# agent-charon/MinGraph-UNet

Hardware: AMD Instinct MI355X
Metric: segmented Mpix/sec, full MinGraph-UNet forward (U-Net + patch-graph GAT), 512x512 batch (higher is better)
Workload: dtype f32

## Files before the change

include/mgunet.h:

```cpp
#ifndef MGUNET_H
#define MGUNET_H

#include <stddef.h>
#include <stdint.h>

#ifdef __cplusplus
extern "C" {
#endif

#define MGU_OK 0
#define MGU_ERR_INVALID -1
#define MGU_ERR_HIP -2
#define MGU_ERR_STATE -3
#define MGU_ERR_NOMEM -4

#define MGU_DTYPE_F32 0
#define MGU_DTYPE_BF16 1

typedef struct mgu_ctx mgu_ctx;

typedef struct {
  const char* name;
  const void* ptr;
  int64_t numel;
// ... 318 lines not shown
int mgu_refine_probs(mgu_ctx* ctx, const float* src_dev, int is_prob, const uint8_t* guide_dev, int B, int H, int W, int C, int G, int radius,
                     const int32_t* space_lut, const int32_t* range_lut, int shift, int iterations, float* probs_dev, int64_t* labels_dev,
                     float* conf_dev, int64_t* changed_dev, void* hip_stream);
int mgu_slic_labels(mgu_ctx* ctx, const uint8_t* rgb_dev, int B, int H, int W, int step, int mq, int passes, const uint16_t* lin_host,
                    const int32_t* m_host, const uint16_t* f_host, int32_t* raw_labels_dev, int32_t* centres_dev, void* hip_stream);
int mgu_regions_connect(mgu_ctx* ctx, const int32_t* raw_labels_dev, int B, int H, int W, int min_area, int rounds, int32_t* labels_dev,
                        int64_t* counts_dev, int64_t* offsets_dev, void* hip_stream);
int mgu_regions_adjacency(mgu_ctx* ctx, const int32_t* labels_dev, const int64_t* offsets_dev, int B, int H, int W, int64_t node_capacity,
                          int64_t edge_capacity, int32_t* rowptr_dev, int32_t* col_dev, int32_t* border_dev, int32_t* status_dev,
                          void* hip_stream);
int mgu_regions_features_u8(mgu_ctx* ctx, const uint8_t* rgb_dev, const int32_t* labels_dev, const int64_t* offsets_dev, int B, int H, int W,
                            const uint16_t* lin_host, const int32_t* m_host, const uint16_t* f_host, int64_t node_capacity, float* feat_dev,
                            int64_t* stats_dev, void* hip_stream);
int mgu_regions_pool_nhwc(mgu_ctx* ctx, const float* feat_dev, int ld, int c_off, int D, const int32_t* labels_dev, const int64_t* offsets_dev,
                          int B, int H, int W, int64_t node_capacity, float* out_dev, void* hip_stream);
int mgu_patch_node_features_u8(mgu_ctx* ctx, const uint8_t* rgb_dev, int B, int H, int W, int patch, const float* img_dev, int64_t is_n,
                               int64_t is_c, int64_t is_h, int64_t is_w, int repeat, const float* unet_rows_dev, int unet_cols, int per_channel,
                               float* out_dev, int ld_out, void* hip_stream);
int mgu_patch_labels(mgu_ctx* ctx, const void* src_dev, int src_kind, int B, int H, int W, int C, int patch, int32_t* counts_dev,
                     int64_t* labels_dev, float* purity_dev, void* hip_stream);
int mgu_graphcut_rev_index(mgu_ctx* ctx, const int64_t* coo_dev, int64_t E, int num_nodes, const int32_t* rowptr_dev, const int32_t* col_dev,
                           int32_t* rev_dev, int32_t* perm_dev, int* status_dev, void* hip_stream);
int mgu_graphcut_capacities(mgu_ctx* ctx, int B, int N, const int64_t* coo_dev, int64_t E, const float* prior_dev, const int32_t* counts_dev,
                            int num_classes, int fg_class, const float* intensity_dev, const float* feat_dev, int D, float gamma,
                            float sigma_intensity, float sigma_features, float smoothness, float unit, int32_t* cap_source_dev,
                            int32_t* cap_sink_dev, int32_t* cap_edge_dev, void* hip_stream);
int mgu_graphcut_solve(mgu_ctx* ctx, int B, int N, int64_t E, const int32_t* rowptr_dev, const int32_t* col_dev, const int32_t* rev_dev,
                       const int32_t* perm_dev, const int32_t* cap_source_dev, const int32_t* cap_sink_dev, const int32_t* cap_edge_dev,
                       int max_rounds, int relabel_period, int threads, uint8_t* labels_dev, int64_t* flow_dev, int32_t* rounds_dev,
                       int32_t* converged_dev, void* hip_stream);
int mgu_graphcut_energy(mgu_ctx* ctx, int B, int N, const int64_t* coo_dev, int64_t E, const uint8_t* labels_dev, const int32_t* cap_source_dev,
                        const int32_t* cap_sink_dev, const int32_t* cap_edge_dev, int64_t* energy_dev, void* hip_stream);
int mgu_graphcut_label_costs(mgu_ctx* ctx, int64_t rows, int K, const float* prob_dev, const int32_t* counts_dev, float unit, int32_t* costs_dev,
                             void* hip_stream);
int mgu_graphcut_expand(mgu_ctx* ctx, int B, int N, int64_t E, int K, const int32_t* rowptr_dev, const int32_t* col_dev, const int32_t* rev_dev,
                        const int32_t* perm_dev, const int32_t* costs_dev, const int32_t* cap_edge_dev, const uint8_t* init_dev, int max_cycles,
                        int max_rounds, int relabel_period, int threads, uint8_t* labels_dev, int64_t* energy_dev, int32_t* moves_dev,
                        int32_t* accepted_dev, int32_t* rounds_dev, int32_t* converged_dev, void* hip_stream);
int mgu_graphcut_energy_multi(mgu_ctx* ctx, int B, int N, const int64_t* coo_dev, int64_t E, int K, const uint8_t* labels_dev, const int32_t* costs_dev,
                              const int32_t* cap_edge_dev, int64_t* energy_dev, void* hip_stream);
int mgu_colorize_labels(mgu_ctx* ctx, const int64_t* labels_dev, int64_t npix, const uint8_t* palette_dev, int num_classes, uint8_t* vis_dev,
                        uint8_t* labels_u8_dev, void* hip_stream);

int mgu_channel_affine_nhwc(mgu_ctx* ctx, const float* x_dev, int ldx, int64_t M, int C, const float* scale_dev,
                            const float* shift_dev, int act, float* y_dev, int ldy, void* hip_stream);
int mgu_channel_sum_nhwc(mgu_ctx* ctx, const float* x_dev, int ldx, int64_t M, int C, float* out_dev, void* hip_stream);

int mgu_channel_sum_images_nhwc(mgu_ctx* ctx, const float* x_dev, int ldx, int B, int64_t M, int C, float* out_dev, void* hip_stream);

int mgu_frame_sad_tile(void);
int mgu_frame_shifts(mgu_ctx* ctx, const uint8_t* frames_u8, int T, int H, int W, int channels, int bgr, int radius, int factor,
                     int32_t* shifts_dev, int64_t* cost_dev, int64_t* surface_dev, void* hip_stream);
int mgu_track_align(mgu_ctx* ctx, const int32_t* labels_dev, const int64_t* offsets_dev, int64_t capacity, const int32_t* shifts_dev, int T,
                    int H, int W, int32_t* prev_aligned_dev, int32_t* next_cropped_dev, int64_t* vis_prev_dev, int64_t* vis_next_dev,
                    void* hip_stream);
int mgu_track_ids(mgu_ctx* ctx, const int64_t* offsets_dev, int T, int64_t capacity, const int64_t* link_dev, const int64_t* class_dev,
                  const int64_t* first_ids_dev, int64_t* next_id_dev, int64_t* track_id_dev, int32_t* track_len_dev, int64_t* track_class_dev,
                  int64_t track_capacity, int32_t* status_dev, void* hip_stream);

int mgu_mask_runs(mgu_ctx* ctx, const int32_t* labels_dev, const int64_t* offsets_dev, int64_t capacity, int B, int H, int W,
                  int64_t run_capacity, int64_t* run_ptr_dev, int32_t* run_start_dev, int32_t* run_length_dev, int32_t* status_dev,
                  void* hip_stream);
int mgu_runs_to_labels(mgu_ctx* ctx, const int64_t* run_ptr_dev, const int32_t* run_start_dev, const int32_t* run_length_dev,
                       int64_t run_capacity, const int64_t* offsets_dev, int64_t capacity, int B, int H, int W, int32_t* labels_dev,
                       int32_t* status_dev, void* hip_stream);
int mgu_object_outlines(mgu_ctx* ctx, const int32_t* labels_dev, const int64_t* offsets_dev, int64_t capacity, int B, int H, int W,
                        int connectivity, int64_t loop_capacity, int64_t vertex_capacity, int64_t* loop_ptr_dev, int64_t* vertex_ptr_dev,
                        int32_t* vertices_dev, int64_t* loop_area2_dev, int32_t* status_dev, void* hip_stream);
int mgu_polygons_to_labels(mgu_ctx* ctx, const int64_t* loop_ptr_dev, const int64_t* vertex_ptr_dev, const int32_t* vertices_dev,
                           int64_t loop_capacity, int64_t vertex_capacity, const int64_t* offsets_dev, int64_t capacity, int B, int H, int W,
                           int frac_bits, int64_t crossing_capacity, int32_t* labels_dev, int32_t* status_dev, void* hip_stream);

double mgu_unet_flops(mgu_ctx* ctx, int B, int H, int W);
double mgu_unet_mfma_flops(mgu_ctx* ctx, int B, int H, int W);
int mgu_profile_enable(mgu_ctx* ctx, int on);
typedef struct {
  const char* name;
  double ms, flops_alg, flops_mfma;
  int launches, pipe;
} mgu_kernel_stat;
int mgu_profile_read_kernels(mgu_ctx* ctx, mgu_kernel_stat* out, int cap, int* n_out);
int mgu_profile_read(mgu_ctx* ctx, double* conv_ms, int* conv_launches, double* total_ms);
int64_t mgu_convt_asm_launches(mgu_ctx* ctx);

#ifdef __cplusplus
}
#endif
#endif
```

mingraph-unet_amd/csrc/common.h:

```cpp
#pragma once
#include <hip/hip_runtime.h>
#include <stdint.h>

#include "device.h"

namespace mgu {

inline int grid_for(int64_t work, int threads, int cap) {
  int64_t b = (work + threads - 1) / threads;
  if (b < 1) b = 1;
  if (b > cap) b = cap;
  return (int)b;
}
inline bool aligned16(const void* p) { return ((uintptr_t)p & 15) == 0; }

struct Tuning {
  bool first_mfma = true;
  bool use_wino = true;
  int wino_prec = 1;
  bool convt_frag = true;
  bool wino_cp = true;
  int wino_ppb_cap = 32;
  bool wgrad_halo = true;
  bool wino_wgrad = true;
  bool convt_dgrad_x3 = true;
  bool wgrad_x3 = true;
  bool wgrad_thin = true;
  bool wino_dgrad = true;
  bool gat_fused = true;
  bool head_fused = true;
  bool wino_asm = true;
  bool convt_asm = true;
  int fwd_groups = 2;
  int lovasz_passes = 4;
};
const Tuning& default_tuning();
hipError_t ensure_dyn_lds(const void* func, size_t bytes, bool (&done)[64]);

struct IgemmDesc {
  const Tuning* tn;
  const float* in;
  const float* w;
  const float* wu;
  const float* scale;
  const float* shift;
  float* out;
  int M;
  int H, W;
  int Cp;
  int ldin;
  int KS;
  int K;
  int Kp;
  int N;
  int ldout;
  int coff;
  int relu;
  int out_mode;
  int ct_cout;
  int Hout, Wout;
  float* pool;
  int ldpool;
  double* stat_slots;
  int split_n;
  float* out2;
  int ld2;
};

struct WinoHead {
  const float* w;
  const float* b;
  float* logits;
  float* psum;
  int ncls;
  int psum_bytes;
};
inline size_t wino_head_psum_bytes(int B, int H, int W) { return (size_t)B * (H / 16) * (W / 16) * 8 * 32 * sizeof(float); }

inline const Tuning& tun(const IgemmDesc& d) { return d.tn ? *d.tn : default_tuning(); }
enum class ConvKernel {
  None,
  WinoAsmWide, WinoAsmCp1r2, WinoAsmCp1r4,
  WinoAsmCp1r2Head,
  WinoCp2, WinoCp1, WinoCp2Stats, WinoCp1Stats,
  WinoCp1Head,
  WinoF32Wide, WinoF32Narrow,
  WinoX3Wide, WinoX3Narrow,
  HaloF32, HaloBf16Np8, HaloBf16Np4,
  TilesF32, TilesBf16,
  ConvtX3, ConvtBf16f, ConvtX3Dgrad,
  ConvtX3Asm,
};
ConvKernel pick_conv(const IgemmDesc& d, int dtype, const WinoHead* head = nullptr);
hipError_t launch_conv(const IgemmDesc& d, ConvKernel k, int dtype, hipStream_t s, const WinoHead* head = nullptr);
inline bool conv_fuses_head(ConvKernel k) { return k == ConvKernel::WinoAsmCp1r2Head || k == ConvKernel::WinoCp1Head; }
inline hipError_t launch_igemm_f32(const IgemmDesc& d, hipStream_t s) { return launch_conv(d, pick_conv(d, 0), 0, s); }
inline hipError_t launch_igemm_bf16(const IgemmDesc& d, hipStream_t s) { return launch_conv(d, pick_conv(d, 1), 1, s); }
const char* conv_kernel_name(ConvKernel k, const IgemmDesc& d);
const char* conv_dgrad_name(ConvKernel k, const IgemmDesc& d);
struct ConvCost {
  double mfma;
  int pipe;
};
ConvCost conv_cost(ConvKernel k, const IgemmDesc& d);
inline bool conv_is_wino(ConvKernel k) { return k >= ConvKernel::WinoAsmWide && k <= ConvKernel::WinoX3Narrow; }
inline bool conv_fuses_pool(ConvKernel k) {
  return conv_is_wino(k) || (k >= ConvKernel::HaloF32 && k <= ConvKernel::HaloBf16Np4);
}
inline bool conv_reads_panel(ConvKernel k) {
  return !conv_is_wino(k) && k != ConvKernel::ConvtX3 && k != ConvKernel::ConvtX3Asm && k != ConvKernel::ConvtBf16f &&
         k != ConvKernel::ConvtX3Dgrad;
}
inline bool conv_reads_convt_x3(ConvKernel k) {
  return k == ConvKernel::ConvtX3 || k == ConvKernel::ConvtX3Asm;
}
bool wino_layer(const Tuning& t, int KS, int Cp);
// ... 165 lines not shown
```

mingraph-unet_amd/csrc/ctx.h:

```cpp
#pragma once
#include <stdarg.h>
#include <stdio.h>
#include <stdlib.h>
#include <string.h>

#include <map>
#include <string>
#include <vector>

#include "../../include/mgunet.h"
#include "common.h"

struct Layer {
  std::string prefix;
  std::string conv;
  std::string bn;
  int Cin = 0, Cp = 0, Cout = 0, KS = 3;
  bool convt = false;
  int K = 0, Kp = 0, N = 0, Np = 0;
  float *wp = nullptr, *scale = nullptr, *shift = nullptr;
  bool first = false;
  bool ctb = false;
  bool ctx3 = false;
  bool wino = false;
// ... 17 lines not shown
  int ldin = 0;
  float* z = nullptr;
  float* y = nullptr;
  int ldy = 0;
  int B = 0, H = 0, W = 0;
};

struct Block {
  int up = -1;
  int conv1 = 0, conv2 = 0;
  int level = 0;
};

struct mgu_ctx {
  int device = 0;
  mgu::Tuning tn;
  std::string err;
  bool configured = false, loaded = false;
  std::vector<mgu::PackBatch> pack_host;
  mgu::PackBatch* pack_dev = nullptr;
  int pack_dev_cap = 0;
  bool want_train = false;
  bool fold_dirty = false;
  int* err_word = nullptr;
  void* redws = nullptr;
  size_t redws_bytes = 0;
  void* pm_out = nullptr;
  int pm_patch = 0;
  void* pmws = nullptr;
  size_t pmws_bytes = 0;
  void* wuws = nullptr;
  size_t wuws_bytes = 0;
  unsigned long long* gmaxbuf = nullptr;
  int gmax_cap = 0;
  unsigned gmax_gen = 0;
  struct mgu_gat_weights* gat_tmp = nullptr;
  void* lossws = nullptr;
  size_t lossws_bytes = 0;
  void* optws = nullptr;
  size_t optws_bytes = 0;
  void* imgws = nullptr;
  size_t imgws_bytes = 0;
  void* ncws = nullptr;
  size_t ncws_bytes = 0;
  void* objws = nullptr;
  size_t objws_bytes = 0;
  void* labtab = nullptr;
  std::vector<unsigned char> labtab_host;
  int in_ch = 0, ncls = 0, feat = 0, depth = 0, dtype = 0, Cp0 = 0;
  std::vector<Layer> layers;
  std::vector<Block> enc, dec;
  Block bott;
  int head = 0;
  int64_t nparams = 0;
  float* arena = nullptr;
  size_t arena_floats = 0;
  void* ws = nullptr;
  size_t ws_bytes = 0;
  void* gbws = nullptr;
  size_t gbws_bytes = 0;
  void* gws = nullptr;
  size_t gws_bytes = 0;
  void* tws = nullptr;
  size_t tws_bytes = 0;
  bool have_train_fwd = false;
  int tB = 0, tH = 0, tW = 0;
  std::vector<FwdRecord> fwd;
  void* comm = nullptr;
  int comm_world = 1, comm_rank = 0;
  hipStream_t comm_stream = nullptr;
  hipEvent_t comm_ev[16] = {};
  int comm_ev_next = 0;
  bool prof = false;
  std::vector<hipEvent_t> ev;
  struct ProfRec {
    const char* name;
    double alg, mfma;
    int pipe;
  };
  std::vector<ProfRec> prec;
  int ev_used = 0;
  hipEvent_t ev_total[2] = {nullptr, nullptr};
  hipStream_t fwd_stream = nullptr;
  hipEvent_t fwd_ev[2] = {nullptr, nullptr};
  int64_t convt_asm_launches = 0;
  int panel_packs = 0;
};

namespace mgud {

inline int rup(int v, int m) { return (v + m - 1) / m * m; }
extern std::string g_create_err;

inline Layer make_layer(int dtype, int Cin, int Cp, int Cout, int KS, bool convt) {
  Layer L;
  L.Cin = Cin, L.Cp = Cp, L.Cout = Cout, L.KS = KS, L.convt = convt;
  L.K = KS * KS * Cp, L.Kp = rup(L.K, dtype == MGU_DTYPE_BF16 ? 64 : 32);
  L.N = convt ? 4 * Cout : Cout, L.Np = rup(L.N, 128);
  return L;
}

inline int fail(mgu_ctx* c, int code, const char* fmt, ...) {
  char buf[512];
  va_list ap;
  va_start(ap, fmt);
  vsnprintf(buf, sizeof buf, fmt, ap);
  va_end(ap);
  if (c) c->err = buf; else g_create_err = buf;
  return code;
}

#define HIPCHK(c, call)                                                                                       \
  do {                                                                                                        \
    hipError_t e_ = (call);                                                                                   \
    if (e_ != hipSuccess) return mgud::fail(c, MGU_ERR_HIP, "%s failed: %s", #call, hipGetErrorString(e_));   \
  } while (0)

inline int ensure(mgu_ctx* c, void** p, size_t* have, size_t need) {
  if (*have >= need) return MGU_OK;
  if (*p) {
    HIPCHK(c, hipDeviceSynchronize());
    HIPCHK(c, hipFree(*p));
    *p = nullptr;
    *have = 0;
  }
  hipError_t e = hipMalloc(p, need);
  if (e != hipSuccess) return fail(c, MGU_ERR_NOMEM, "hipMalloc(%zu) failed: %s", need, hipGetErrorString(e));
  *have = need;
  return MGU_OK;
}

inline int err_word_dev(mgu_ctx* c, int** dev) {
  if (!c->err_word) {
    HIPCHK(c, hipHostMalloc((void**)&c->err_word, sizeof(int), hipHostMallocMapped));
    *c->err_word = 0;
  }
  HIPCHK(c, hipHostGetDevicePointer((void**)dev, c->err_word, 0));
  return MGU_OK;
}
inline const char* err_word_message(int w) {
  return (w & 2) ? "the GAT backward found no edge whose score equals the forward's graph-wide maximum (mgu_gat_layer_backward): its "
                   "max term was not applied"
                 : "a label outside [0, num_classes) (and != ignore_index -100) reached a loss kernel of this context (mgu_cross_entropy / "
                   "mgu_dice_loss; F.one_hot / CrossEntropyLoss raise on it)";
}

struct Carve {
  size_t off = 0;
  size_t take(size_t bytes) {
    const size_t o = off;
    off += (bytes + 255) / 256 * 256;
    return o;
  }
};

struct ProfScope {
  mgu_ctx* c;
  hipStream_t s;
  int idx = -1;
  ProfScope(mgu_ctx* c_, hipStream_t s_, const char* name = "conv/GEMM", double alg = 0, double mfma = 0, int pipe = -1) : c(c_), s(s_) {
    if (!c || !c->prof) return;
    if ((size_t)c->ev_used >= c->prec.size()) c->prec.resize(c->ev_used + 1);
    c->prec[c->ev_used] = {name, alg, mfma, pipe};
    if ((size_t)(2 * c->ev_used + 2) > c->ev.size()) {
      hipEvent_t a, b;
      if (hipEventCreate(&a) != hipSuccess || hipEventCreate(&b) != hipSuccess) return;
      c->ev.push_back(a);
// ... 141 lines not shown
```

mingraph-unet_amd/csrc/mgunet_api.hip:

```cpp
#include "ctx.h"

#include <algorithm>

using namespace mgu;
using namespace mgud;

namespace mgud {
std::string g_create_err;
}

namespace {

struct WsPlan {
  size_t xin, tmp, tmp_slice, bott, total;
  std::vector<size_t> pooled;
};

int fwd_groups(const mgu_ctx* c, int B) { return c->tn.fwd_groups >= 2 && B >= 2 ? 2 : 1; }
int group_images(const mgu_ctx* c, int B) { return (B + fwd_groups(c, B) - 1) / fwd_groups(c, B); }

WsPlan plan_ws(const mgu_ctx* c, int B, int H, int W) {
  std::vector<int> hs, wsz;
  level_dims(H, W, c->depth, hs, wsz);
  auto out = [&](const Block& b, int l) { return (size_t)B * hs[l] * wsz[l] * c->layers[b.conv2].Cout; };
  WsPlan p;
  Carve k;
  const size_t es = c->dtype == MGU_DTYPE_BF16 ? 2 : 4;
  p.xin = k.take((size_t)B * H * W * c->Cp0 * es);
  size_t tmax = out(c->bott, c->bott.level);
  for (const Block& b : c->enc) tmax = std::max(tmax, out(b, b.level));
  const int G = fwd_groups(c, B);
  p.tmp_slice = (tmax / B * group_images(c, B) * es + 255) / 256 * 256;
  p.tmp = k.take(G == 1 ? tmax * es : G * p.tmp_slice);
  for (const Block& b : c->enc) p.pooled.push_back(k.take(out(b, b.level + 1) * es));
  p.bott = k.take(out(c->bott, c->bott.level) * es);
  p.total = k.off;
  return p;
}

template <class F>
void weight_forms(const mgu_ctx* c, Layer& L, F form) {
  const int dtype = c->dtype;
  L.wino = dtype == MGU_DTYPE_F32 && !L.convt && wino_layer(c->tn, L.KS, L.Cp);
  L.ctx3 = dtype == MGU_DTYPE_F32 && L.convt && convt_x3_layer(c->tn, L.Cin, L.Cout);
  L.ctb = dtype == MGU_DTYPE_BF16 && L.convt && convt_bf16f_layer(c->tn, L.Cin, L.Cout);
  L.first = !L.convt && L.KS == 3 && first_conv_applicable(dtype, L.Cin, L.Cp, L.Cout, 8, 0);
  form(L.wp, (size_t)L.Np * L.Kp);
  form(L.scale, (size_t)L.Np);
  form(L.shift, (size_t)L.Np);
  if (L.wino) form(L.wu, wino_u_floats(L.Cout, L.Cp));
  if (L.wino && rup(L.Cout, 4) % 16 == 0) form(L.wug, wino_u_floats(L.Cin, rup(L.Cout, 4)));
  if (L.ctx3) form(L.wu, convt_x3_floats(L.Cin, L.Cout));
  if (L.ctb) form(L.wu, convt_bf16f_floats(L.Cin, L.Cout));
  if (L.ctx3) form(L.wxg, convt_x3_dgrad_floats(L.Cin, L.Cout));
  if (dtype == MGU_DTYPE_F32 && !L.convt && L.bn.empty())
    form(L.wxg, (size_t)rup(L.Cin, 128) * rup(L.KS * L.KS * rup(L.Cout, 4), 32));
  if (L.first) form(L.wf, 9 * 4 * (size_t)L.Cout);
  if (L.first) form(L.wfm, first_mfma_floats());
  if (!L.bn.empty()) {
    form(L.mean, (size_t)L.Np);
    form(L.invstd, (size_t)L.Np);
    form(L.tscale, (size_t)L.Np);
    form(L.tshift, (size_t)L.Np);
  }
}

}

extern "C" {

const char* mgu_version(void) { return "mgunet 0.2 (gfx950: fp32 Winograd / bf16 MFMA forward, fp32 training step, GAT, RCCL gradient exchange)"; }

int mgu_create(int device_id, mgu_ctx** out) {
  if (!out) return fail(nullptr, MGU_ERR_INVALID, "out == NULL");
  int n = 0;
  hipError_t e = hipGetDeviceCount(&n);
  if (e != hipSuccess || n <= 0)
    return fail(nullptr, MGU_ERR_HIP, "no HIP device available (%s): libmgunet has no CPU fallback",
                e != hipSuccess ? hipGetErrorString(e) : "device count 0");
  if (device_id < 0 || device_id >= n) return fail(nullptr, MGU_ERR_INVALID, "device %d out of range [0,%d)", device_id, n);
  e = hipSetDevice(device_id);
  if (e != hipSuccess) return fail(nullptr, MGU_ERR_HIP, "hipSetDevice: %s", hipGetErrorString(e));
  mgu_ctx* c = new mgu_ctx();
  c->device = device_id;
  auto flag = [](const char* name) { const char* v = getenv(name); return v && v[0] == '1'; };
  auto num = [](const char* name, int dflt) { const char* v = getenv(name); return v && v[0] ? atoi(v) : dflt; };
  Tuning& t = c->tn;
  t.first_mfma = !flag("MGU_NO_FIRST_MFMA");
  t.use_wino = !flag("MGU_NO_WINOGRAD");
  t.wino_prec = num("MGU_WINO_PREC", t.wino_prec) ? 1 : 0;
  t.wino_cp = !flag("MGU_NO_WINO_CP");
  t.convt_frag = !flag("MGU_NO_CONVT_FRAG");
  t.wino_ppb_cap = std::max(1, num("MGU_WINO_PPB_CAP", 32));
  t.wgrad_halo = !flag("MGU_NO_WGRAD_HALO");
  t.wino_wgrad = !flag("MGU_NO_WINO_WGRAD");
  t.wgrad_x3 = !flag("MGU_NO_WGRAD_X3");
  t.convt_dgrad_x3 = !flag("MGU_NO_CONVT_DGRAD_X3");
  t.wgrad_thin = !flag("MGU_NO_THIN_WGRAD");
  t.wino_dgrad = !flag("MGU_NO_WINO_DGRAD");
  t.gat_fused = !flag("MGU_NO_GAT_FUSED");
  t.wino_asm = num("MGU_WINO_ASM", 1) > 0;
  t.convt_asm = num("MGU_CONVT_ASM", 1) > 0;
  t.head_fused = num("MGU_HEAD_FUSED", 1) > 0;
  t.fwd_groups = num("MGU_FWD_GROUPS", t.fwd_groups) >= 2 ? 2 : 1;
  t.lovasz_passes = num("MGU_LOVASZ_PASSES", t.lovasz_passes) == 3 ? 3 : 4;
  *out = c;
  return MGU_OK;
}

void mgu_destroy(mgu_ctx* c) {
  if (!c) return;
  (void)hipSetDevice(c->device);
  (void)hipDeviceSynchronize();
  (void)mgu_comm_destroy(c);
  if (c->arena) (void)hipFree(c->arena);
  if (c->ws) (void)hipFree(c->ws);
  if (c->gws) (void)hipFree(c->gws);
  if (c->pmws) (void)hipFree(c->pmws);
  if (c->gbws) (void)hipFree(c->gbws);
  if (c->pack_dev) (void)hipFree(c->pack_dev);
  if (c->tws) (void)hipFree(c->tws);
  if (c->redws) (void)hipFree(c->redws);
  if (c->wuws) (void)hipFree(c->wuws);
  if (c->ncws) (void)hipFree(c->ncws);
  if (c->objws) (void)hipFree(c->objws);
  if (c->labtab) (void)hipFree(c->labtab);
  if (c->lossws) (void)hipFree(c->lossws);
  if (c->imgws) (void)hipFree(c->imgws);
  if (c->optws) (void)hipFree(c->optws);
  gat_destroy(c);
  if (c->err_word) (void)hipHostFree(c->err_word);
  for (auto e : c->ev) (void)hipEventDestroy(e);
  for (auto e : c->ev_total)
    if (e) (void)hipEventDestroy(e);
  for (auto e : c->fwd_ev)
    if (e) (void)hipEventDestroy(e);
  if (c->fwd_stream) (void)hipStreamDestroy(c->fwd_stream);
  delete c;
}

const char* mgu_last_error(mgu_ctx* c) { return c ? c->err.c_str() : g_create_err.c_str(); }

int mgu_unet_configure(mgu_ctx* c, int in_ch, int ncls, int feat, int depth, int dtype) {
  if (!c) return MGU_ERR_INVALID;
  if (in_ch < 1 || ncls < 1 || feat < 4 || (feat & 3) || depth < 1 || depth > 8)
    return fail(c, MGU_ERR_INVALID, "unsupported UNet(%d,%d,%d,%d): init_features must be a positive multiple of 4, depth 1..8",
                in_ch, ncls, feat, depth);
  if (dtype != MGU_DTYPE_F32 && dtype != MGU_DTYPE_BF16) return fail(c, MGU_ERR_INVALID, "unknown dtype %d", dtype);
  if (dtype == MGU_DTYPE_BF16 && ((feat & 7) || ncls > 4))
    return fail(c, MGU_ERR_INVALID, "bf16 storage needs init_features %% 8 == 0 (16-byte lanes of 8 bf16) and <= 4 classes");
  HIPCHK(c, hipSetDevice(c->device));
  c->in_ch = in_ch, c->ncls = ncls, c->feat = feat, c->depth = depth, c->dtype = dtype;
  c->Cp0 = rup(in_ch, dtype == MGU_DTYPE_BF16 ? 8 : 4);
  c->layers.clear();
  c->enc.clear();
  c->dec.clear();
  auto add = [&](const std::string& prefix, const char* conv, const char* bn, int cin, int cp, int cout, int KS, bool convt, int level) {
    Layer L = make_layer(dtype, cin, cp, cout, KS, convt);
    L.prefix = prefix, L.conv = conv, L.bn = bn, L.level = level;
    c->layers.push_back(L);
    return (int)c->layers.size() - 1;
  };
  auto add_block = [&](const std::string& prefix, int cin, int cp, int cout, int level, int up) {
    Block b;
    b.up = up, b.level = level;
    b.conv1 = add(prefix, "conv1", "bn1", cin, cp, cout, 3, false, level);
    b.conv2 = add(prefix, "conv2", "bn2", cout, cout, cout, 3, false, level);
    return b;
  };
  int cin = in_ch, cp = c->Cp0, f = feat;
  for (int i = 0; i < depth; ++i) {
    c->enc.push_back(add_block("encoder.encoder_blocks." + std::to_string(i) + ".", cin, cp, f, i, -1));
    cin = cp = f;
    f *= 2;
  }
  c->bott = add_block("encoder.bottleneck.", cin, cp, f, depth, -1);
  int prev = f;
  for (int b = 0; b < depth; ++b) {
    const int i = depth - 1 - b, ci = feat << i;
    const std::string prefix = "decoder.decoder_blocks." + std::to_string(b) + ".";
    const int up = add(prefix, "upsample", "", prev, prev, prev / 2, 1, true, i + 1);
    c->dec.push_back(add_block(prefix + "conv_block.", ci + prev / 2, ci + prev / 2, ci, i, up));
    prev = ci;
  }
  c->head = add("decoder.", "final_conv", "", prev, prev, ncls, 1, false, 0);
  c->fwd.assign(c->layers.size(), FwdRecord{});
  {
    int64_t off = 0;
    auto conv = [&](Layer& L) {
      L.off_w = off, off += (int64_t)L.Cout * L.Cin * L.KS * L.KS * (L.convt ? 4 : 1);
      L.off_b = off, off += L.Cout;
    };
    auto bn = [&](Layer& L) {
      L.off_gamma = off, off += L.Cout;
      L.off_beta = off, off += L.Cout;
    };
    auto block = [&](const Block& b) {
      if (b.up >= 0) conv(c->layers[b.up]);
      conv(c->layers[b.conv1]), conv(c->layers[b.conv2]);
      bn(c->layers[b.conv1]), bn(c->layers[b.conv2]);
    };
    for (const Block& b : c->enc) block(b);
    block(c->bott);
    for (const Block& b : c->dec) block(b);
    conv(c->layers[c->head]);
    c->nparams = off;
  }
  size_t total = 0;
  for (auto& L : c->layers) weight_forms(c, L, [&](float*&, size_t n) { total += n; });
  if (c->arena) HIPCHK(c, hipFree(c->arena));
  c->arena = nullptr;
  HIPCHK(c, hipMalloc((void**)&c->arena, total * sizeof(float)));
  HIPCHK(c, hipMemset(c->arena, 0, total * sizeof(float)));
  c->arena_floats = total;
  float* p = c->arena;
  for (auto& L : c->layers) weight_forms(c, L, [&](float*& form, size_t n) { form = p, p += n; });
  c->configured = true;
  c->have_train_fwd = false;
  c->loaded = false;
// ... 188 lines not shown
  if (took) *took = t;
  if (L.wp_dirty && conv_reads_panel(k)) {
    HIPCHK(c, launch_pack_one(L.convt ? pack_convt_panel(L.w_src, L.wp, c->dtype, L.Cin, L.Cout, L.Kp)
                                      : pack_conv_panel(L.w_src, L.wp, c->dtype, L.Cout, L.Cin, L.Cp, L.KS, L.Kp), s));
    L.wp_dirty = false;
    ++c->panel_packs;
  }
  double alg = L.convt ? 2.0 * d.M * (double)L.Cin * L.Cout * 4.0 : 2.0 * d.M * (double)L.KS * L.KS * L.Cin * L.Cout;
  if (head) alg += 2.0 * d.M * (double)L.Cout * head->ncls;
  const ConvCost cost = conv_cost(k, d);
  ProfScope ps(c, s, conv_kernel_name(k, d), alg, cost.mfma, cost.pipe);
  HIPCHK(c, launch_conv(d, k, c->dtype, s, head));
  c->convt_asm_launches += k == ConvKernel::ConvtX3Asm;
  return MGU_OK;
}

extern "C" {

int mgu_unet_forward(mgu_ctx* c, const void* x_dev, int B, int H, int W, int64_t xs_n, int64_t xs_c, int64_t xs_h,
                     int64_t xs_w, void* logits_dev, void* const* cat_dev, void* const* feat_dev, int training,
                     void* hip_stream) {
  if (!c) return MGU_ERR_INVALID;
  if (!c->configured || !c->loaded) return fail(c, MGU_ERR_STATE, "configure + load_weights must precede forward");
  if (!x_dev || !logits_dev || !cat_dev || !feat_dev) return fail(c, MGU_ERR_INVALID, "NULL buffer");
  const int depth = c->depth;
  if (B < 1 || H < (1 << depth) || W < (1 << depth))
    return fail(c, MGU_ERR_INVALID, "input %dx%dx%d too small for depth %d", B, H, W, depth);
  if ((int64_t)B * H * W >= (1ll << 31)) return fail(c, MGU_ERR_INVALID, "B*H*W must be < 2^31");
  for (int i = 0; i < depth; ++i)
    if (!cat_dev[i] || !feat_dev[i]) return fail(c, MGU_ERR_INVALID, "NULL cat/feat buffer %d", i);
  HIPCHK(c, hipSetDevice(c->device));
  hipStream_t s = (hipStream_t)hip_stream;
  if (training && c->dtype != MGU_DTYPE_F32)
    return fail(c, MGU_ERR_STATE, "training runs in fp32 only (bf16 storage is an inference mode)");
  if (training) {
    int rc = unet_forward_train(c, (const float*)x_dev, xs_n, xs_c, xs_h, xs_w, B, H, W, (float*)logits_dev, cat_dev, feat_dev, s);
    if (rc == MGU_OK && c->pm_out) {
      ProfScope ps(c, s, "patch_mean_kernel", 0, 0, -1);
      HIPCHK(c, launch_patch_mean(feat_dev[0], 0, (float*)c->pm_out, B, H, W, c->feat, c->pm_patch, s));
      c->pm_out = nullptr;
    }
    return rc;
  }
  const WsPlan plan = plan_ws(c, B, H, W);
  int rc = ensure(c, &c->ws, &c->ws_bytes, plan.total);
  if (rc) return rc;
  const Layer& F = c->layers[c->head];
  WinoHead head_args{};
  bool head_done = false;
  const bool head_wanted = c->pm_out && F.w_src && F.b_src && wino_head_layer(c->tn, c->dtype, F.Cin, c->ncls, c->pm_patch, B, H, W);
  if (head_wanted) {
    if ((rc = ensure(c, &c->pmws, &c->pmws_bytes, wino_head_psum_bytes(B, H, W)))) return rc;
    head_args = WinoHead{F.w_src, F.b_src, (float*)logits_dev, (float*)c->pmws, c->ncls, (int)wino_head_psum_bytes(B, H, W)};
  }
  if (c->fold_dirty) {
    for (auto& L : c->layers)
      if (!L.bn.empty()) HIPCHK(c, launch_bn_fold(L.b_src, L.gamma, L.beta, L.run_mean, L.run_var, 1e-5f, L.scale, L.shift, L.Cout, s));
    c->fold_dirty = false;
  }
  char* ws = (char*)c->ws;
  const size_t es = c->dtype == MGU_DTYPE_BF16 ? 2 : 4;
  void* xin = ws + plan.xin;
  void* bott = ws + plan.bott;
  std::vector<int> hs, wsz;
  level_dims(H, W, depth, hs, wsz);

  if (c->prof) {
    for (auto& e : c->ev_total)
      if (!e) HIPCHK(c, hipEventCreate(&e));
    HIPCHK(c, hipEventRecord(c->ev_total[0], s));
  }

  for (const Block& b : c->enc) {
    const int i = b.level;
    if (2 * hs[i + 1] != hs[i] || 2 * wsz[i + 1] != wsz[i])
      HIPCHK(c, hipMemsetAsync(cat_dev[i], 0, (size_t)B * hs[i] * wsz[i] * 2 * c->layers[b.conv2].Cout * es, s));
  }

  const Layer& L0 = c->layers[c->enc[0].conv1];
  const bool first_direct = L0.wfm && c->tn.first_mfma && first_mfma_applicable(c->dtype, L0.Cin, L0.Cp, L0.Cout, c->feat, 0, H, W) &&
                            (int64_t)B * H * W < (1ll << 31);
  if (!first_direct) HIPCHK(c, launch_pack_input((const float*)x_dev, xin, c->dtype, B, c->in_ch, c->Cp0, H, W, xs_n, xs_c, xs_h, xs_w, s));

  auto walk = [&](hipStream_t gs, int img0, int nb, void* tmp, bool* head_done) -> int {
    auto at = [&](const void* base, int level, int ch) { return (char*)base + (size_t)img0 * hs[level] * wsz[level] * ch * es; };
    WinoHead head = head_args;
    if (head_wanted) {
      head.logits += (size_t)img0 * H * W * c->ncls;
      head.psum = (float*)((char*)head.psum + wino_head_psum_bytes(img0, H, W));
      head.psum_bytes = (int)wino_head_psum_bytes(nb, H, W);
    }
    auto conv = [&](int l, int lvl, ConvReq q, const ConvFusions& f = {}, ConvTaken* took = nullptr) {
      const Layer& L = c->layers[l];
      q.B = nb, q.H = hs[lvl], q.W = wsz[lvl], q.scale = L.bn.empty() ? nullptr : L.scale, q.shift = L.shift;
      return run_layer(c, L, q, gs, f, took);
    };
    const void* cur = at(xin, 0, c->Cp0);
    int cur_ld = c->Cp0;
    for (const Block& b : c->enc) {
      const int i = b.level, C = c->layers[b.conv1].Cout;
      if (&b == &c->enc.front() && first_direct) {
        if (c->fold_dirty) return fail(c, MGU_ERR_STATE, "internal: eval scale/shift not folded");
        const double alg = 2.0 * nb * H * W * 9.0 * L0.Cin * L0.Cout;
        ProfScope ps(c, gs, "conv3x3_first_mfma_kernel", alg, 2.0 * nb * H * W * 32.0 * 32.0 * (c->dtype == MGU_DTYPE_F32 ? 6.0 : 3.0), 1);
        HIPCHK(c, launch_first_mfma_direct(c->dtype, (const float*)x_dev + (int64_t)img0 * xs_n, xs_n, xs_c, xs_h, xs_w, c->in_ch, L0.wfm,
                                           L0.bn.empty() ? nullptr : L0.scale, L0.shift, tmp, nb, H, W, C, 0, 1, gs));
      } else if ((rc = conv(b.conv1, i, {.in = cur, .ldin = cur_ld, .out = tmp, .ldout = C, .relu = 1}))) return rc;
      void *cat = at(cat_dev[i], i, 2 * C), *pooled = at(ws + plan.pooled[i], i + 1, C);
      ConvTaken took;
      if ((rc = conv(b.conv2, i, {.in = tmp, .ldin = C, .out = cat, .ldout = 2 * C, .relu = 1}, {.pool = pooled, .ldpool = C}, &took))) return rc;
      if (!took.pool) {
        ProfScope ps(c, gs, "maxpool2", 0, 0, -1);
        HIPCHK(c, launch_maxpool2(cat, 2 * C, pooled, c->dtype, nb, hs[i], wsz[i], C, gs));
      }
      cur = pooled, cur_ld = C;
    }
    {
      const Block& b = c->bott;
      const int i = b.level, C = c->layers[b.conv1].Cout;
      if ((rc = conv(b.conv1, i, {.in = cur, .ldin = cur_ld, .out = tmp, .ldout = C, .relu = 1}))) return rc;
      if ((rc = conv(b.conv2, i, {.in = tmp, .ldin = C, .out = at(bott, i, C), .ldout = C, .relu = 1}))) return rc;
      cur = at(bott, i, C), cur_ld = C;
    }
    for (const Block& b : c->dec) {
      const int i = b.level, C = c->layers[b.conv1].Cout;
      const bool last = head_wanted && i == 0;
      void *cat = at(cat_dev[i], i, 2 * C), *feat = at(feat_dev[i], i, C);
      if ((rc = conv(b.up, i + 1, {.in = cur, .ldin = cur_ld, .out = cat, .ldout = 2 * C, .coff = C, .Hout = hs[i], .Wout = wsz[i]}))) return rc;
      if ((rc = conv(b.conv1, i, {.in = cat, .ldin = 2 * C, .out = tmp, .ldout = C, .relu = 1}))) return rc;
      ConvTaken took;
      if ((rc = conv(b.conv2, i, {.in = tmp, .ldin = C, .out = feat, .ldout = C, .relu = 1}, {.head = last ? &head : nullptr}, &took))) return rc;
      if (last) *head_done = took.head;
      cur = feat, cur_ld = C;
    }
    return MGU_OK;
  };
  const int G = c->prof ? 1 : fwd_groups(c, B);
  if (G == 1) {
    if ((rc = walk(s, 0, B, ws + plan.tmp, &head_done))) return rc;
  } else {
    if (!c->fwd_stream) HIPCHK(c, hipStreamCreateWithFlags(&c->fwd_stream, hipStreamNonBlocking));
    for (auto& e : c->fwd_ev)
      if (!e) HIPCHK(c, hipEventCreateWithFlags(&e, hipEventDisableTiming));
    const int n0 = group_images(c, B), packs = c->panel_packs;
    bool done1 = false;
    HIPCHK(c, hipEventRecord(c->fwd_ev[0], s));
    HIPCHK(c, hipStreamWaitEvent(c->fwd_stream, c->fwd_ev[0], 0));
    rc = walk(s, 0, n0, ws + plan.tmp, &head_done);
    if (rc == MGU_OK && c->panel_packs != packs) {
      HIPCHK(c, hipEventRecord(c->fwd_ev[0], s));
      HIPCHK(c, hipStreamWaitEvent(c->fwd_stream, c->fwd_ev[0], 0));
    }
    const int rc1 = rc == MGU_OK ? walk(c->fwd_stream, n0, B - n0, ws + plan.tmp + plan.tmp_slice, &done1) : MGU_OK;
    HIPCHK(c, hipEventRecord(c->fwd_ev[1], c->fwd_stream));
    HIPCHK(c, hipStreamWaitEvent(s, c->fwd_ev[1], 0));
    if (rc || rc1) return rc ? rc : rc1;
    if (done1 != head_done) return fail(c, MGU_ERR_STATE, "internal: the image groups disagree on the head-fused kernel");
  }
  const void* cur = feat_dev[0];
  const int cur_ld = c->layers[c->dec.back().conv1].Cout;
  {
    const int pm_dtype = c->dtype;
    if (head_done) {
      ProfScope ps(c, s, "patch_sum_combine_kernel", 0, 0, -1);
      HIPCHK(c, launch_patch_sum_combine((const float*)c->pmws, (float*)c->pm_out, B * (H / 16) * (W / 16), s));
      c->pm_out = nullptr;
    } else if (c->pm_out && F.w_src && F.b_src && patch_mean_head_fusable(pm_dtype, F.Cin, c->ncls) && F.Cin <= 256) {
      ProfScope ps(c, s, "patch_mean_kernel (1x1 head + patch means)", 2.0 * B * H * W * F.Cin * c->ncls, 0, -1);
      HIPCHK(c, launch_patch_mean(cur, pm_dtype, (float*)c->pm_out, B, H, W, F.Cin, c->pm_patch, s, F.w_src, F.b_src,
                                  (float*)logits_dev, c->ncls));
      c->pm_out = nullptr;
    } else if (c->ncls <= 4 && F.w_src && F.b_src) {
      ProfScope ps(c, s, "conv1x1_head_kernel", 2.0 * B * H * W * F.Cin * c->ncls, 0, -1);
      HIPCHK(c, launch_conv1x1_head(cur, c->dtype, cur_ld, F.Cin, F.w_src, F.b_src, (float*)logits_dev, c->ncls, c->ncls,
                                    (int64_t)B * H * W, s));
    } else if ((rc = run_layer(c, F, {.in = cur, .ldin = cur_ld, .B = B, .H = H, .W = W, .out = logits_dev, .ldout = c->ncls, .shift = F.shift}, s))) {
      return rc;
    }
  }
  if (c->pm_out) {
    ProfScope ps(c, s, "patch_mean_kernel", 0, 0, -1);
    HIPCHK(c, launch_patch_mean(cur, c->dtype, (float*)c->pm_out, B, H, W, F.Cin, c->pm_patch, s));
    c->pm_out = nullptr;
  }
  if (c->prof) HIPCHK(c, hipEventRecord(c->ev_total[1], s));
  return MGU_OK;
}

int mgu_unet_request_patch_mean(mgu_ctx* c, int patch, void* out_dev) {
  if (!c) return MGU_ERR_INVALID;
  if (!c->configured) return fail(c, MGU_ERR_STATE, "not configured");
  if (!out_dev) {
    c->pm_out = nullptr;
    return MGU_OK;
  }
  if (patch < 1) return fail(c, MGU_ERR_INVALID, "bad patch_mean request");
  const int C = c->layers[c->head].Cin, vec = c->dtype == MGU_DTYPE_BF16 ? 8 : 4;
  if ((C % vec) || C > 256) return fail(c, MGU_ERR_INVALID, "patch means need init_features %% %d == 0 and <= 256 (got %d)", vec, C);
  c->pm_patch = patch;
  c->pm_out = out_dev;
  return MGU_OK;
}

struct mgu_conv_weights {
  Layer L;
};

static int conv2d_launch(mgu_ctx* c, const Layer& L, const void* in_dev, int B, int H, int W, const void* bias_dev, const void* scale_dev,
                         const void* shift_dev, int relu, void* out_dev, int ld_out, int c_off, hipStream_t s) {
  IgemmDesc d = layer_desc(c, L, in_dev, L.Cin, B, H, W, out_dev, ld_out, c_off);
  d.relu = relu;
  if (scale_dev && shift_dev) {
    d.scale = (const float*)scale_dev;
    d.shift = (const float*)shift_dev;
  } else if (bias_dev) {
    HIPCHK(c, launch_pack_one(pack_bias_tile((const float*)bias_dev, L.shift, L.Cout, 1), s));
    d.shift = L.shift;
  }
  const ConvKernel k = pick_conv(d, 0);
  ProfScope ps(c, s, conv_kernel_name(k, d));
  HIPCHK(c, launch_conv(d, k, 0, s));
  return MGU_OK;
}

int mgu_conv2d_prepare(mgu_ctx* c, const void* w_dev, int Cout, int Cin, int ksize, mgu_conv_weights** out, void* hip_stream) {
  if (!c) return MGU_ERR_INVALID;
  if (!w_dev || !out || Cout < 1 || (ksize != 1 && ksize != 3)) return fail(c, MGU_ERR_INVALID, "bad conv2d_prepare args (ksize must be 1 or 3)");
  if (Cin < 4 || (Cin & 3)) return fail(c, MGU_ERR_INVALID, "conv2d needs Cin %% 4 == 0 (got %d)", Cin);
  HIPCHK(c, hipSetDevice(c->device));
  hipStream_t s = (hipStream_t)hip_stream;
  mgu_conv_weights* p = new mgu_conv_weights();
  Layer& L = p->L;
  L = make_layer(MGU_DTYPE_F32, Cin, Cin, Cout, ksize, false);
  const bool wino = wino_layer(c->tn, ksize, Cin);
  const size_t panel = (size_t)L.Np * L.Kp, total = panel + L.Np + (wino ? wino_u_floats(Cout, Cin) : 0);
  hipError_t e = hipMalloc((void**)&L.wp, total * sizeof(float));
  if (e != hipSuccess) {
    delete p;
    return fail(c, MGU_ERR_NOMEM, "hipMalloc(%zu) failed: %s", total * sizeof(float), hipGetErrorString(e));
  }
  L.shift = L.wp + panel;
  e = hipMemsetAsync(L.wp, 0, (panel + L.Np) * sizeof(float), s);
  if (e == hipSuccess) e = launch_pack_one(pack_conv_panel((const float*)w_dev, L.wp, 0, Cout, Cin, Cin, ksize, L.Kp), s);
  if (e == hipSuccess && wino) {
    L.wu = L.shift + L.Np;
    e = launch_pack_one(pack_wino((const float*)w_dev, L.wu, Cout, Cin, Cin, 0, c->tn.wino_prec), s);
  }
  if (e != hipSuccess) {
// ... 82 lines not shown
  HIPCHK(c, launch_conv(d, k, 0, s));
  c->convt_asm_launches += k == ConvKernel::ConvtX3Asm;
  return MGU_OK;
}

int mgu_maxpool2x2_nhwc(mgu_ctx* c, const void* in_dev, int ld_in, int B, int H, int W, int Cc, void* out_dev,
                        void* hip_stream) {
  if (!c) return MGU_ERR_INVALID;
  if (!in_dev || !out_dev || B < 1 || H < 2 || W < 2 || Cc < 4 || (Cc & 3) || ld_in < Cc || (ld_in & 3))
    return fail(c, MGU_ERR_INVALID, "bad maxpool args (C and ld_in must be multiples of 4, H,W >= 2)");
  HIPCHK(c, hipSetDevice(c->device));
  HIPCHK(c, launch_maxpool2(in_dev, ld_in, out_dev, 0, B, H, W, Cc, (hipStream_t)hip_stream));
  return MGU_OK;
}

int mgu_argmax_classes(mgu_ctx* c, const void* logits_dev, int64_t npix, int num_classes, int64_t* pred_dev,
                       void* hip_stream) {
  if (!c || !logits_dev || !pred_dev || num_classes < 1 || npix < 0) return fail(c, MGU_ERR_INVALID, "bad argmax args");
  HIPCHK(c, hipSetDevice(c->device));
  HIPCHK(c, launch_argmax((const float*)logits_dev, npix, num_classes, pred_dev, (hipStream_t)hip_stream));
  return MGU_OK;
}

int mgu_patch_mean(mgu_ctx* c, const void* feat_dev, int feat_dtype, int B, int H, int W, int C, int patch, void* out_dev,
                   void* hip_stream) {
  if (!c || !feat_dev || !out_dev || B < 1 || H < 1 || W < 1 || patch < 1)
    return fail(c, MGU_ERR_INVALID, "bad patch_mean args");
  if (feat_dtype != MGU_DTYPE_F32 && feat_dtype != MGU_DTYPE_BF16) return fail(c, MGU_ERR_INVALID, "unknown dtype %d", feat_dtype);
  const int vec = feat_dtype == MGU_DTYPE_BF16 ? 8 : 4;
  if ((C % vec) || C < vec || C > 256)
    return fail(c, MGU_ERR_INVALID, "patch_mean needs C %% %d == 0 and C <= 256 (got %d)", vec, C);
  HIPCHK(c, hipSetDevice(c->device));
  HIPCHK(c, launch_patch_mean(feat_dev, feat_dtype, (float*)out_dev, B, H, W, C, patch, (hipStream_t)hip_stream));
  return MGU_OK;
}

static double net_flops(const mgu_ctx* c, int B, int H, int W, bool mfma) {
  std::vector<int> hs, wsz;
  level_dims(H, W, c->depth, hs, wsz);
  double fl = 0;
  for (const Layer& L : c->layers) {
    const int h = hs[L.level], w = wsz[L.level];
    if (mfma && L.wino) fl += 2.0 * ((h + 1) / 2) * ((w + 1) / 2) * 16.0 * L.Cp * L.Cout;
    else fl += 2.0 * h * w * L.KS * L.KS * L.Cin * L.Cout * (L.convt ? 4.0 : 1.0);
  }
  return fl * B;
}

double mgu_unet_flops(mgu_ctx* c, int B, int H, int W) { return c && c->configured ? net_flops(c, B, H, W, false) : -1.0; }

double mgu_unet_mfma_flops(mgu_ctx* c, int B, int H, int W) { return c && c->configured ? net_flops(c, B, H, W, true) : -1.0; }

int mgu_profile_enable(mgu_ctx* c, int on) {
  if (!c) return MGU_ERR_INVALID;
  c->prof = on != 0;
  c->ev_used = 0;
  return MGU_OK;
}

int mgu_profile_read_kernels(mgu_ctx* c, mgu_kernel_stat* out, int cap, int* n_out) {
  if (!c || !n_out || (cap > 0 && !out)) return MGU_ERR_INVALID;
  int n = 0;
  for (int i = 0; i < c->ev_used; ++i) {
    float ms = 0;
    HIPCHK(c, hipEventSynchronize(c->ev[2 * i + 1]));
    HIPCHK(c, hipEventElapsedTime(&ms, c->ev[2 * i], c->ev[2 * i + 1]));
    const mgu_ctx::ProfRec& r = c->prec[i];
    int k = 0;
    while (k < n && strcmp(out[k].name, r.name) != 0) ++k;
    if (k == n) {
      if (n == cap) continue;
      out[n].name = r.name, out[n].ms = 0, out[n].flops_alg = 0, out[n].flops_mfma = 0, out[n].launches = 0, out[n].pipe = r.pipe;
      ++n;
    }
    out[k].ms += ms, out[k].flops_alg += r.alg, out[k].flops_mfma += r.mfma, out[k].launches += 1;
  }
  *n_out = n;
  c->ev_used = 0;
  return MGU_OK;
}

int64_t mgu_convt_asm_launches(mgu_ctx* c) { return c ? c->convt_asm_launches : 0; }

int mgu_profile_read(mgu_ctx* c, double* conv_ms, int* conv_launches, double* total_ms) {
  if (!c) return MGU_ERR_INVALID;
  if (c->ev_used == 0 || !c->ev_total[1]) return fail(c, MGU_ERR_STATE, "no profiled forward to read");
  HIPCHK(c, hipEventSynchronize(c->ev_total[1]));
  double sum = 0;
  for (int i = 0; i < c->ev_used; ++i) {
    float ms = 0;
    HIPCHK(c, hipEventSynchronize(c->ev[2 * i + 1]));
    HIPCHK(c, hipEventElapsedTime(&ms, c->ev[2 * i], c->ev[2 * i + 1]));
    sum += ms;
  }
  float tot = 0;
  HIPCHK(c, hipEventElapsedTime(&tot, c->ev_total[0], c->ev_total[1]));
  if (conv_ms) *conv_ms = sum;
  if (conv_launches) *conv_launches = c->ev_used;
  if (total_ms) *total_ms = tot;
  return MGU_OK;
}

}
```

Before: 836.8.

## Make the image-group stream split configurable per U-Net stage and split patch combine

Replaces the single forward walk with a list of stages (encoder levels, bottleneck, decoder levels), each with its own one- or two-group setting from a per-stage plan. Consecutive stages with the same setting run together, either on one stream or split across two streams with fork/join events. The patch-sum combine kernel now runs per image group inside the final split run, so it can overlap with the other stream. With the default plan every stage is split in two, so the schedule is mostly the old one except for the per-group combine. The change adds event bookkeeping and complexity in exchange for future per-stage tuning.

After: 839.7 (median of 3 runs). Within noise of the previous version (+0.4%).

```diff
diff --git a/include/mgunet.h b/include/mgunet.h
--- a/include/mgunet.h
+++ b/include/mgunet.h
@@ -424,6 +424,7 @@
 int mgu_profile_read_kernels(mgu_ctx* ctx, mgu_kernel_stat* out, int cap, int* n_out);
 int mgu_profile_read(mgu_ctx* ctx, double* conv_ms, int* conv_launches, double* total_ms);
 int64_t mgu_convt_asm_launches(mgu_ctx* ctx);
+int64_t mgu_patch_combine_launches(mgu_ctx* ctx);
 
 #ifdef __cplusplus
 }
diff --git a/mingraph-unet_amd/csrc/common.h b/mingraph-unet_amd/csrc/common.h
--- a/mingraph-unet_amd/csrc/common.h
+++ b/mingraph-unet_amd/csrc/common.h
@@ -31,7 +31,8 @@
   bool head_fused = true;
   bool wino_asm = true;
   bool convt_asm = true;
-  int fwd_groups = 2;
+  static constexpr int FWD_STAGES = 9;
+  unsigned char fwd_plan[FWD_STAGES] = {2, 2, 2, 2, 2, 2, 2, 2, 2};
   int lovasz_passes = 4;
 };
 const Tuning& default_tuning();
diff --git a/mingraph-unet_amd/csrc/ctx.h b/mingraph-unet_amd/csrc/ctx.h
--- a/mingraph-unet_amd/csrc/ctx.h
+++ b/mingraph-unet_amd/csrc/ctx.h
@@ -123,7 +123,8 @@
   int ev_used = 0;
   hipEvent_t ev_total[2] = {nullptr, nullptr};
   hipStream_t fwd_stream = nullptr;
-  hipEvent_t fwd_ev[2] = {nullptr, nullptr};
+  std::vector<hipEvent_t> fwd_ev;
+  int64_t patch_combine_launches = 0;
   int64_t convt_asm_launches = 0;
   int panel_packs = 0;
 };
diff --git a/mingraph-unet_amd/csrc/mgunet_api.hip b/mingraph-unet_amd/csrc/mgunet_api.hip
--- a/mingraph-unet_amd/csrc/mgunet_api.hip
+++ b/mingraph-unet_amd/csrc/mgunet_api.hip
@@ -16,7 +16,19 @@
   std::vector<size_t> pooled;
 };
 
-int fwd_groups(const mgu_ctx* c, int B) { return c->tn.fwd_groups >= 2 && B >= 2 ? 2 : 1; }
+int fwd_plan_index(int depth, int level, bool decoder) {
+  if (level >= depth) return 4;
+  const int l = std::min(level, 3);
+  return decoder ? 8 - l : l;
+}
+int stage_groups(const mgu_ctx* c, int B, int level, bool decoder) {
+  return B >= 2 && c->tn.fwd_plan[fwd_plan_index(c->depth, level, decoder)] >= 2 ? 2 : 1;
+}
+int fwd_groups(const mgu_ctx* c, int B) {
+  int g = stage_groups(c, B, c->depth, false);
+  for (int l = 0; l < c->depth; ++l) g = std::max({g, stage_groups(c, B, l, false), stage_groups(c, B, l, true)});
+  return g;
+}
 int group_images(const mgu_ctx* c, int B) { return (B + fwd_groups(c, B) - 1) / fwd_groups(c, B); }
 
 WsPlan plan_ws(const mgu_ctx* c, int B, int H, int W) {
@@ -102,7 +114,16 @@
   t.wino_asm = num("MGU_WINO_ASM", 1) > 0;
   t.convt_asm = num("MGU_CONVT_ASM", 1) > 0;
   t.head_fused = num("MGU_HEAD_FUSED", 1) > 0;
-  t.fwd_groups = num("MGU_FWD_GROUPS", t.fwd_groups) >= 2 ? 2 : 1;
+  if (const char* v = getenv("MGU_FWD_GROUPS"); v && v[0])
+    for (auto& g : t.fwd_plan) g = atoi(v) >= 2 ? 2 : 1;
+  if (const char* v = getenv("MGU_FWD_PLAN"); v && v[0]) {
+    if (strlen(v) != (size_t)Tuning::FWD_STAGES || strspn(v, "12") != (size_t)Tuning::FWD_STAGES) {
+      delete c;
+      return fail(nullptr, MGU_ERR_INVALID, "MGU_FWD_PLAN='%s': expected %d characters '1' or '2' (encoder levels 0-3, bottleneck, decoder "
+                  "blocks on levels 3-0)", v, Tuning::FWD_STAGES);
+    }
+    for (int i = 0; i < Tuning::FWD_STAGES; ++i) t.fwd_plan[i] = (unsigned char)(v[i] - '0');
+  }
   t.lovasz_passes = num("MGU_LOVASZ_PASSES", t.lovasz_passes) == 3 ? 3 : 4;
   *out = c;
   return MGU_OK;
@@ -133,8 +154,7 @@
   for (auto e : c->ev) (void)hipEventDestroy(e);
   for (auto e : c->ev_total)
     if (e) (void)hipEventDestroy(e);
-  for (auto e : c->fwd_ev)
-    if (e) (void)hipEventDestroy(e);
+  for (auto e : c->fwd_ev) (void)hipEventDestroy(e);
   if (c->fwd_stream) (void)hipStreamDestroy(c->fwd_stream);
   delete c;
 }
@@ -489,7 +509,29 @@
                             (int64_t)B * H * W < (1ll << 31);
   if (!first_direct) HIPCHK(c, launch_pack_input((const float*)x_dev, xin, c->dtype, B, c->in_ch, c->Cp0, H, W, xs_n, xs_c, xs_h, xs_w, s));
 
-  auto walk = [&](hipStream_t gs, int img0, int nb, void* tmp, bool* head_done) -> int {
+  struct Stage {
+    const Block* b;
+    const void* in;
+    int in_level, in_ld, groups;
+  };
+  std::vector<Stage> stages;
+  {
+    auto groups = [&](int level, bool decoder) { return c->prof ? 1 : stage_groups(c, B, level, decoder); };
+    const void* cur = xin;
+    int cur_level = 0, cur_ld = c->Cp0;
+    for (const Block& b : c->enc) {
+      stages.push_back({&b, cur, cur_level, cur_ld, groups(b.level, false)});
+      cur = ws + plan.pooled[b.level], cur_level = b.level + 1, cur_ld = c->layers[b.conv1].Cout;
+    }
+    stages.push_back({&c->bott, cur, cur_level, cur_ld, groups(depth, false)});
+    cur = bott, cur_ld = c->layers[c->bott.conv1].Cout;
+    for (const Block& b : c->dec) {
+      stages.push_back({&b, cur, cur_level, cur_ld, groups(b.level, true)});
+      cur = feat_dev[b.level], cur_level = b.level, cur_ld = c->layers[b.conv1].Cout;
+    }
+  }
+
+  auto run_stage = [&](const Stage& st, hipStream_t gs, int img0, int nb, void* tmp, bool* head_done) -> int {
     auto at = [&](const void* base, int level, int ch) { return (char*)base + (size_t)img0 * hs[level] * wsz[level] * ch * es; };
     WinoHead head = head_args;
     if (head_wanted) {
@@ -502,10 +544,10 @@
       q.B = nb, q.H = hs[lvl], q.W = wsz[lvl], q.scale = L.bn.empty() ? nullptr : L.scale, q.shift = L.shift;
       return run_layer(c, L, q, gs, f, took);
     };
-    const void* cur = at(xin, 0, c->Cp0);
-    int cur_ld = c->Cp0;
-    for (const Block& b : c->enc) {
-      const int i = b.level, C = c->layers[b.conv1].Cout;
+    const Block& b = *st.b;
+    const void* cur = at(st.in, st.in_level, st.in_ld);
+    const int cur_ld = st.in_ld, i = b.level, C = c->layers[b.conv1].Cout;
+    if (b.up < 0 && i < depth) {
       if (&b == &c->enc.front() && first_direct) {
         if (c->fold_dirty) return fail(c, MGU_ERR_STATE, "internal: eval scale/shift not folded");
         const double alg = 2.0 * nb * H * W * 9.0 * L0.Cin * L0.Cout;
@@ -520,17 +562,10 @@
         ProfScope ps(c, gs, "maxpool2", 0, 0, -1);
         HIPCHK(c, launch_maxpool2(cat, 2 * C, pooled, c->dtype, nb, hs[i], wsz[i], C, gs));
       }
-      cur = pooled, cur_ld = C;
-    }
-    {
-      const Block& b = c->bott;
-      const int i = b.level, C = c->layers[b.conv1].Cout;
+    } else if (b.up < 0) {
       if ((rc = conv(b.conv1, i, {.in = cur, .ldin = cur_ld, .out = tmp, .ldout = C, .relu = 1}))) return rc;
       if ((rc = conv(b.conv2, i, {.in = tmp, .ldin = C, .out = at(bott, i, C), .ldout = C, .relu = 1}))) return rc;
-      cur = at(bott, i, C), cur_ld = C;
-    }
-    for (const Block& b : c->dec) {
-      const int i = b.level, C = c->layers[b.conv1].Cout;
+    } else {
       const bool last = head_wanted && i == 0;
       void *cat = at(cat_dev[i], i, 2 * C), *feat = at(feat_dev[i], i, C);
       if ((rc = conv(b.up, i + 1, {.in = cur, .ldin = cur_ld, .out = cat, .ldout = 2 * C, .coff = C, .Hout = hs[i], .Wout = wsz[i]}))) return rc;
@@ -538,39 +573,62 @@
       ConvTaken took;
       if ((rc = conv(b.conv2, i, {.in = tmp, .ldin = C, .out = feat, .ldout = C, .relu = 1}, {.head = last ? &head : nullptr}, &took))) return rc;
       if (last) *head_done = took.head;
-      cur = feat, cur_ld = C;
     }
     return MGU_OK;
   };
-  const int G = c->prof ? 1 : fwd_groups(c, B);
-  if (G == 1) {
-    if ((rc = walk(s, 0, B, ws + plan.tmp, &head_done))) return rc;
-  } else {
-    if (!c->fwd_stream) HIPCHK(c, hipStreamCreateWithFlags(&c->fwd_stream, hipStreamNonBlocking));
-    for (auto& e : c->fwd_ev)
-      if (!e) HIPCHK(c, hipEventCreateWithFlags(&e, hipEventDisableTiming));
-    const int n0 = group_images(c, B), packs = c->panel_packs;
-    bool done1 = false;
-    HIPCHK(c, hipEventRecord(c->fwd_ev[0], s));
-    HIPCHK(c, hipStreamWaitEvent(c->fwd_stream, c->fwd_ev[0], 0));
-    rc = walk(s, 0, n0, ws + plan.tmp, &head_done);
-    if (rc == MGU_OK && c->panel_packs != packs) {
-      HIPCHK(c, hipEventRecord(c->fwd_ev[0], s));
-      HIPCHK(c, hipStreamWaitEvent(c->fwd_stream, c->fwd_ev[0], 0));
-    }
-    const int rc1 = rc == MGU_OK ? walk(c->fwd_stream, n0, B - n0, ws + plan.tmp + plan.tmp_slice, &done1) : MGU_OK;
-    HIPCHK(c, hipEventRecord(c->fwd_ev[1], c->fwd_stream));
-    HIPCHK(c, hipStreamWaitEvent(s, c->fwd_ev[1], 0));
-    if (rc || rc1) return rc ? rc : rc1;
-    if (done1 != head_done) return fail(c, MGU_ERR_STATE, "internal: the image groups disagree on the head-fused kernel");
+  const int nodes_per_image = (H / 16) * (W / 16);
+  auto combine = [&](hipStream_t gs, int img0, int nb) -> int {
+    ProfScope ps(c, gs, "patch_sum_combine_kernel", 0, 0, -1);
+    HIPCHK(c, launch_patch_sum_combine((const float*)((const char*)c->pmws + wino_head_psum_bytes(img0, H, W)),
+                                       (float*)c->pm_out + (size_t)img0 * nodes_per_image * 32, nb * nodes_per_image, gs));
+    ++c->patch_combine_launches;
+    return MGU_OK;
+  };
+  const int n0 = group_images(c, B);
+  bool combined = false;
+  for (size_t k = 0, run = 0; k < stages.size(); ++run) {
+    size_t k1 = k;
+    while (k1 < stages.size() && stages[k1].groups == stages[k].groups) ++k1;
+    const bool tail = k1 == stages.size();
+    if (stages[k].groups == 1) {
+      for (size_t j = k; j < k1; ++j)
+        if ((rc = run_stage(stages[j], s, 0, B, ws + plan.tmp, &head_done))) return rc;
+    } else {
+      if (!c->fwd_stream) HIPCHK(c, hipStreamCreateWithFlags(&c->fwd_stream, hipStreamNonBlocking));
+      while (c->fwd_ev.size() < 2 * run + 2) {
+        hipEvent_t e;
+        HIPCHK(c, hipEventCreateWithFlags(&e, hipEventDisableTiming));
+        c->fwd_ev.push_back(e);
+      }
+      const hipEvent_t fork = c->fwd_ev[2 * run], join = c->fwd_ev[2 * run + 1];
+      const int packs = c->panel_packs;
+      bool done1 = false;
+      HIPCHK(c, hipEventRecord(fork, s));
+      HIPCHK(c, hipStreamWaitEvent(c->fwd_stream, fork, 0));
+      for (size_t j = k; j < k1 && rc == MGU_OK; ++j) rc = run_stage(stages[j], s, 0, n0, ws + plan.tmp, &head_done);
+      if (rc == MGU_OK && tail && head_done) rc = combine(s, 0, n0);
+      if (rc == MGU_OK && c->panel_packs != packs) {
+        HIPCHK(c, hipEventRecord(fork, s));
+        HIPCHK(c, hipStreamWaitEvent(c->fwd_stream, fork, 0));
+      }
+      int rc1 = MGU_OK;
+      for (size_t j = k; j < k1 && rc == MGU_OK && rc1 == MGU_OK; ++j)
+        rc1 = run_stage(stages[j], c->fwd_stream, n0, B - n0, ws + plan.tmp + plan.tmp_slice, &done1);
+      if (rc == MGU_OK && rc1 == MGU_OK && tail && done1) rc1 = combine(c->fwd_stream, n0, B - n0);
+      HIPCHK(c, hipEventRecord(join, c->fwd_stream));
+      HIPCHK(c, hipStreamWaitEvent(s, join, 0));
+      if (rc || rc1) return rc ? rc : rc1;
+      if (tail && done1 != head_done) return fail(c, MGU_ERR_STATE, "internal: the image groups disagree on the head-fused kernel");
+      combined = tail && head_done;
+    }
+    k = k1;
   }
   const void* cur = feat_dev[0];
   const int cur_ld = c->layers[c->dec.back().conv1].Cout;
   {
     const int pm_dtype = c->dtype;
     if (head_done) {
-      ProfScope ps(c, s, "patch_sum_combine_kernel", 0, 0, -1);
-      HIPCHK(c, launch_patch_sum_combine((const float*)c->pmws, (float*)c->pm_out, B * (H / 16) * (W / 16), s));
+      if (!combined && (rc = combine(s, 0, B))) return rc;
       c->pm_out = nullptr;
     } else if (c->pm_out && F.w_src && F.b_src && patch_mean_head_fusable(pm_dtype, F.Cin, c->ncls) && F.Cin <= 256) {
       ProfScope ps(c, s, "patch_mean_kernel (1x1 head + patch means)", 2.0 * B * H * W * F.Cin * c->ncls, 0, -1);
@@ -819,6 +877,8 @@
 
 int64_t mgu_convt_asm_launches(mgu_ctx* c) { return c ? c->convt_asm_launches : 0; }
 
+int64_t mgu_patch_combine_launches(mgu_ctx* c) { return c ? c->patch_combine_launches : 0; }
+
 int mgu_profile_read(mgu_ctx* c, double* conv_ms, int* conv_launches, double* total_ms) {
   if (!c) return MGU_ERR_INVALID;
   if (c->ev_used == 0 || !c->ev_total[1]) return fail(c, MGU_ERR_STATE, "no profiled forward to read");
```
